# wangxiaohit/GNNPN-SC

Hardware: AMD Instinct MI355X
Metric: service-composition problems/sec (ML+2PN inference) (higher is better)
Workload: dtype f32-split3xf16 (f32 operands and results; recurrent W_hh.h products: fp32 operands split exactly into 3 x f16, six f16-matrix-core products per term, f32 accumulate; everything else f32 arithmetic)

## Files before the change

gnnpn-sc_amd/csrc/decode_lean.hip:

```cpp
#include "common.h"
#include "recurrent.h"
#include "decode_shared.h"
#include "coop_common.h"
#include "lstm_shared.h"

namespace {
constexpr int H = COOP_H;
constexpr int G = COOP_G;
constexpr int ROWS = COOP_ROWS;
constexpr int UNITS = H / G;
constexpr int KW = 16;
constexpr unsigned SPIN_LIMIT = 400000;
constexpr int XP_GRANULES = ROWS * KW * G;

typedef unsigned u32x2 __attribute__((ext_vector_type(2)));
constexpr int AUX_SC1 = 16;


__device__ __forceinline__ __amdgpu_buffer_rsrc_t make_rsrc(const void* p, unsigned bytes) {
    return __builtin_amdgcn_make_buffer_rsrc(const_cast<void*>(p), 0, (int)bytes, 0x00020000);
}
__device__ __forceinline__ void store_granule(__amdgpu_buffer_rsrc_t r, unsigned voff, unsigned soff, u64 g, bool same_xcd) {
    const u32x2 v = {(unsigned)g, (unsigned)(g >> 32)};
    if (same_xcd) __builtin_amdgcn_raw_buffer_store_b64(v, r, voff, soff, 0);
    else __builtin_amdgcn_raw_buffer_store_b64(v, r, voff, soff, AUX_SC1);
}
}

template <bool SPLIT, int OCC, int EVH, bool DIAG = false>
__global__ __launch_bounds__(256, OCC) void pointer_decode_lean_kernel(DecodeArgs a, u64* xh, u64* xp,
                                                                     u64* xl, unsigned* __restrict__ err,
                                                                     unsigned* __restrict__ sticky, int n_nets, int groups_per_net,
                                                                     int gpx, int flags, unsigned* __restrict__ seats,
                                                                     unsigned* __restrict__ diag) {
    __shared__ __attribute__((aligned(16))) float hs[SPLIT ? 3 * SPLIT_TILE / 2 : ROWS * LDT];
    __shared__ __attribute__((aligned(16))) unsigned wts[SPLIT ? SPLIT_WT_DWORDS : 4];
    __shared__ __attribute__((aligned(16))) float hsl[ROWS][UNITS + 4];
    __shared__ __attribute__((aligned(16))) float win[ROWS][KW][8];
    __shared__ int sel[ROWS];
    __shared__ int abort_flag;
    __shared__ int place[2];

    const int tid = threadIdx.x, lane = tid & 63, wave = __builtin_amdgcn_readfirstlane(tid >> 6);
    const int kq = lane >> 4, c = lane & 15;
    CoopSeat seat;
    if (!coop_enter<G>(err, sticky, seats, gpx, flags, n_nets, groups_per_net, place, &abort_flag, seat)) return;
    const int group = __builtin_amdgcn_readfirstlane(seat.group), member = __builtin_amdgcn_readfirstlane(seat.member);
    const int net_id = __builtin_amdgcn_readfirstlane(seat.net), gi = __builtin_amdgcn_readfirstlane(seat.index_in_net);
    const bool same_xcd = seat.same_xcd;
    const DecodeNet& net = a.net[net_id];

    const int B = a.B, T = a.T, K = a.K, L = T * K;
    const bool latent_in_launch = net.latent_from >= 0;
    const bool has_lat = latent_in_launch || net.latent_win;
    bool publishes_latent = false;
    for (int n = 0; n < n_nets; ++n) publishes_latent |= (a.net[n].latent_from == net_id);
    const bool first = member == 0;

    const int unit = member * UNITS + wave * 8 + (c & 7);
    const int wrow[2] = {(0 + (c >> 3)) * H + unit, (2 + (c >> 3)) * H + unit};
    float wBh[SPLIT ? 1 : 2][SPLIT ? 1 : 64];
    f16x8 wH16[SPLIT ? 2 : 1][8], wL16[SPLIT ? 2 : 1][8];
    float winv[2] = {1.0f, 1.0f};
    unsigned* wt_lane = wts + (SPLIT ? (wave * 8 * 64 + lane) * 4 : 0);
    float bh[2], bi[2], sg[2], wXf[2][2];
    const uint4* __restrict__ Wsplit = SPLIT ? static_cast<const uint4*>(net.whh_split) : nullptr;
    if constexpr (SPLIT) {
        if (Wsplit) load_split_weights(Wsplit + (size_t)member * SPLIT_PACK_U4_PER_MEMBER, tid, wH16, wL16, wt_lane, winv);
    }
#pragma unroll
    for (int tl = 0; tl < 2; ++tl) {
        const int gate = wrow[tl] / H, u = wrow[tl] % H;
        bh[tl] = net.bhh[wrow[tl]];
        if constexpr (SPLIT) {
            if (!Wsplit) winv[tl] = split_weights<H>(net.whh, gate, u, kq, wH16[tl], wL16[tl], wt_lane + 2 * tl);
        } else {
            load_whh_fragments<H>(net.whh, gate, u, kq, wBh[tl]);
        }
        load_folded_input(net.xw_fold, net.xb_fold, wrow[tl], kq, wXf[tl], bi[tl]);
        sg[tl] = net.start_fold[wrow[tl]];
    }

    const int own0 = kq * 4 + (c < 8 ? 0 : 2);
    const int vo_hpub = (int)(own0 * H + unit) * 8u;
    const int vo_sweep = 16 * lane;
    constexpr int VO_NONE = (int)0xFFFFFF00u;
    const int rq = kq, r = c;
    const bool live = r < K;
    const int vo_p = live ? 64 * lane : VO_NONE;
    const int vo_lat = live ? (int)(rq * K + r) * 8u : VO_NONE;
    const int vo_wl = (int)((wave * 4 + rq) * T * K + r) * 4u;
    const int vo_idx = (int)((wave * 4 + rq) * T) * 4u;
    const int vo_act = (int)(c * T * 8 + kq) * 4u;
    const int vo_q = (int)(own0 * T * H + unit) * 4u;
    constexpr int EVN = 8 / EVH;
    const int ppair = tid / EVH, phalf = tid - ppair * EVH;
    const int prow = ppair / K, pcand = ppair - prow * K;
    const bool pdot = ppair < ROWS * K;
    const int vo_ev = pdot ? (int)(((size_t)prow * L + pcand) * H + member * UNITS + phalf * (4 * EVN)) * 4u : VO_NONE;
    const int vo_ppub = (int)((prow * KW + pcand) * G + member) * 8u;
    const int wr_row = tid >> 4, wr_cand = tid & 15;
    const bool wr_live = wr_cand < K;
    const int vo_win = wr_live ? (int)(((size_t)wr_row * L + wr_cand) * 8) * 4u : VO_NONE;

    __amdgpu_buffer_rsrc_t r_h = make_rsrc(xh + (size_t)group * (2 * ROWS * H), 2 * ROWS * H * 8);
    __amdgpu_buffer_rsrc_t r_p = make_rsrc(xp + (size_t)group * (2 * XP_GRANULES), 2 * XP_GRANULES * 8);

    const int n_tiles = (B + ROWS - 1) / ROWS;
    unsigned step = 0;
    unsigned tiles_done = 0;
    for (int tile = gi; tile < n_tiles; tile += groups_per_net) {
        const int b0 = tile * ROWS;
        const int rows_here = min(ROWS, B - b0);
        __amdgpu_buffer_rsrc_t r_enc = make_rsrc(net.enc_out + (size_t)b0 * L * H, (unsigned)((size_t)rows_here * L * H * 4));
        __amdgpu_buffer_rsrc_t r_in = make_rsrc(a.inputs + (size_t)b0 * L * 8, (unsigned)((size_t)rows_here * L * 32));
        __amdgpu_buffer_rsrc_t r_lat = make_rsrc(xl + (size_t)tile * T * ROWS * K, (unsigned)((size_t)T * ROWS * K * 8));
        __amdgpu_buffer_rsrc_t r_wl = make_rsrc(net.win_logits + (size_t)b0 * T * K, (unsigned)((size_t)rows_here * T * K * 4));
        __amdgpu_buffer_rsrc_t r_idx = make_rsrc(net.idx + (size_t)b0 * T, (unsigned)((size_t)rows_here * T * 4));
        __amdgpu_buffer_rsrc_t r_act = make_rsrc(net.actions + (size_t)b0 * T * 8, (unsigned)((size_t)rows_here * T * 32));
        __amdgpu_buffer_rsrc_t r_lw = make_rsrc(net.latent_win ? net.latent_win + (size_t)b0 * T * K : nullptr,
                                                net.latent_win ? (unsigned)((size_t)rows_here * T * K * 4) : 0u);
        __amdgpu_buffer_rsrc_t r_q = make_rsrc(net.queries ? net.queries + (size_t)b0 * T * H : nullptr,
                                               net.queries ? (unsigned)((size_t)rows_here * T * H * 4) : 0u);
        f32x2 cst, hl = {0.f, 0.f};
        cst.x = b0 + own0 < B ? net.c0[(int64_t)(b0 + own0) * H + unit] : 0.0f;
        cst.y = b0 + own0 + 1 < B ? net.c0[(int64_t)(b0 + own0 + 1) * H + unit] : 0.0f;
        __syncthreads();
        for (int j = 0; j < ROWS; ++j) {
            const float h0v = (b0 + j < B) ? net.h0[(int64_t)(b0 + j) * H + tid] : 0.0f;
            if constexpr (SPLIT) split_store(reinterpret_cast<_Float16*>(hs) + j * LDH16 + tid, h0v);
            else hs[ht_index(j, tid)] = h0v;
        }
        __syncthreads();

        for (int k = 0; k <= T; ++k) {
            float axf0 = 0.0f, axf1 = 0.0f;
            u64 st[8] = {0, 0, 0, 0, 0, 0, 0, 0};
            if constexpr (DIAG) st[0] = st[1] = st[2] = st[3] = st[4] = st[5] = phase_stamp();
            const unsigned tag = step;
            const unsigned par = (step - 1) & 1;
            const unsigned so_k = (unsigned)k * (unsigned)K;
            u32x4 ev[EVN];
            u32x4 vp[4];
            u32x2 vl;
#pragma unroll
            for (int j = 0; j < EVN; ++j) asm volatile("" : "=v"(ev[j]));
#pragma unroll
            for (int j = 0; j < 4; ++j) asm volatile("" : "=v"(vp[j]));
            asm volatile("" : "=v"(vl));
            f32x4 ah[2] = {f32x4{0.f, 0.f, 0.f, 0.f}, f32x4{0.f, 0.f, 0.f, 0.f}};

            constexpr bool EV_EARLY = OCC == 1;
            auto request_ev = [&]() {
#pragma unroll
                for (int j = 0; j < EVN; ++j) ev[j] = __builtin_amdgcn_raw_buffer_load_b128(r_enc, vo_ev, so_k * (H * 4) + 16u * j, 0);
            };
            if (k < T) {
                if (k > 0) {
                    const unsigned so_h0 = par * (ROWS * H * 8) + wave * (4 * H * 8);
                    u32x4 vh[8];
                    bool ok = false;
                    unsigned h_miss = 0;
                    for (unsigned spins = 0; spins <= SPIN_LIMIT; ++spins) {
                        unsigned so_h = so_h0;
                        asm volatile("" : "+s"(so_h));
#pragma unroll
                        for (int j = 0; j < 8; ++j) vh[j] = __builtin_amdgcn_raw_buffer_load_b128(r_h, vo_sweep, so_h + 1024u * j, AUX_SC1);
                        bool good = true;
#pragma unroll
                        for (int j = 0; j < 8; ++j) {
                            if constexpr (SPLIT) good &= split_pair_tagged(vh[j], tag);
                            else good &= (vh[j].y == tag) & (vh[j].w == tag);
                        }
                        if (__all(good)) {
                            ok = true;
                            break;
                        }
                        __builtin_amdgcn_s_sleep(1);
                    }
                    if constexpr (DIAG) st[1] = phase_stamp();
                    if (!ok) {
                        abort_flag = 1;
#pragma unroll
                        for (int j = 0; j < 8; ++j) {
                            bool bad;
                            if constexpr (SPLIT) bad = !split_pair_tagged(vh[j], tag);
                            else bad = (vh[j].y != tag) | (vh[j].w != tag);
                            const unsigned long long bm = __ballot(bad);
                            for (int q = 0; q < 4; ++q)
                                if ((bm >> (16 * q)) & 0xffffull) h_miss |= 1u << (4 * (j & 1) + q);
                        }
                        if (lane == 0) coop_failure_record(diag, err, gpx, group, member, tile, k, wave, tag, h_miss, 0u, 0u);
                    }
#pragma unroll
                    for (int j = 0; j < 8; ++j) {
                        const int i = 2 * (j * 64 + lane);
                        if constexpr (SPLIT) {
                            split_pair_to_lds(reinterpret_cast<_Float16*>(hs) + (wave * 4 + (i >> 8)) * LDH16 + (i & 255), vh[j]);
                        } else {
                            float* d = &hs[ht_index(wave * 4 + (i >> 8), i & 255)];
                            d[0] = __uint_as_float(vh[j].x);
                            d[64] = __uint_as_float(vh[j].z);
                        }
                    }
                    if constexpr (EV_EARLY) request_ev();
                    __syncthreads();
                    if (abort_flag) break;
                } else if constexpr (EV_EARLY) {
                    request_ev();
                }
                if constexpr (DIAG) st[2] = phase_stamp();
                constexpr bool EARLY_P = OCC == 1 || !SPLIT;
                auto request_p = [&]() {
                    if (EARLY_P && k > 0) {
                        const unsigned so_p = par * (XP_GRANULES * 8) + wave * (4 * KW * G * 8);
#pragma unroll
                        for (int j = 0; j < 4; ++j) vp[j] = __builtin_amdgcn_raw_buffer_load_b128(r_p, vo_p, so_p + 16u * j, AUX_SC1);
                        if (latent_in_launch)
                            vl = __builtin_amdgcn_raw_buffer_load_b64(r_lat, vo_lat, (unsigned)(((k - 1) * ROWS + wave * 4) * K) * 8u, AUX_SC1);
                    }
                };
                if constexpr (SPLIT) split_chain(reinterpret_cast<const _Float16*>(hs) + c * LDH16 + 8 * kq, wH16, wL16, wt_lane, winv, ah, request_p);
                else mfma_chain_pair<LDT, OCC == 2 ? 8 : 16, true>(hs, c, kq, wBh[0], wBh[SPLIT ? 0 : 1], ah[0], ah[1], request_p);
                if constexpr (DIAG) {
                    asm volatile("" ::"v"(ah[0][0]), "v"(ah[1][0]));
                    st[3] = phase_stamp();
                }
            }

            if (k > 0) {
                const unsigned so_p0 = par * (XP_GRANULES * 8) + wave * (4 * KW * G * 8);
                const unsigned so_l0 = (unsigned)(((k - 1) * ROWS + wave * 4) * K) * 8u;
                bool ok = false;
                for (unsigned spins = 0; spins <= SPIN_LIMIT; ++spins) {
                    if (spins > 0 || k == T || (OCC != 1 && SPLIT)) {
                        unsigned so_p = so_p0, so_l = so_l0;
                        asm volatile("" : "+s"(so_p), "+s"(so_l));
#pragma unroll
                        for (int j = 0; j < 4; ++j) vp[j] = __builtin_amdgcn_raw_buffer_load_b128(r_p, vo_p, so_p + 16u * j, AUX_SC1);
                        if (latent_in_launch) vl = __builtin_amdgcn_raw_buffer_load_b64(r_lat, vo_lat, so_l, AUX_SC1);
                    }
                    bool good = true;
                    if (live) {
#pragma unroll
                        for (int j = 0; j < 4; ++j) good &= (vp[j].y == tag) & (vp[j].w == tag);
                        if (latent_in_launch) good &= vl.y == 1u;
                    }
                    if (__all(good)) {
                        ok = true;
                        break;
                    }
                    __builtin_amdgcn_s_sleep(1);
                }
                if constexpr (DIAG) st[4] = phase_stamp();
                if (!ok) {
                    abort_flag = 1;
                    unsigned p_miss = 0;
#pragma unroll
                    for (int j = 0; j < 4; ++j) {
                        if (__ballot(live && vp[j].y != tag)) p_miss |= 1u << (2 * j);
                        if (__ballot(live && vp[j].w != tag)) p_miss |= 1u << (2 * j + 1);
                    }
                    const unsigned l_miss = (unsigned)__popcll(__ballot(live && latent_in_launch && vl.y != 1u));
                    if (lane == 0) coop_failure_record(diag, err, gpx, group, member, tile, k, wave, tag, 0u, p_miss, l_miss);
                }

                {
                    const int row = wave * 4 + rq;
                    const unsigned so_t = (unsigned)(k - 1) * (unsigned)K * 4u;
                    float dot = 0.0f, lv = 0.0f;
                    if (live) {
                        dot = __fadd_rn(__fadd_rn(__fadd_rn(__uint_as_float(vp[0].x), __uint_as_float(vp[0].z)), __uint_as_float(vp[1].x)), __uint_as_float(vp[1].z));
                        dot = __fadd_rn(__fadd_rn(__fadd_rn(__fadd_rn(dot, __uint_as_float(vp[2].x)), __uint_as_float(vp[2].z)), __uint_as_float(vp[3].x)), __uint_as_float(vp[3].z));
                        if (latent_in_launch) lv = __uint_as_float(vl.x);
                        else if (net.latent_win) lv = __uint_as_float(__builtin_amdgcn_raw_buffer_load_b32(r_lw, vo_wl, so_t, 0));
                    }
                    float v = a.use_tanh ? __fmul_rn(a.tanh_c, tanhf(dot)) : dot;
                    if (live && first) {
                        __builtin_amdgcn_raw_buffer_store_b32(__float_as_uint(v), r_wl, vo_wl, so_t, 0);
                        if (publishes_latent)
                            __builtin_amdgcn_raw_buffer_store_b64(u32x2{__float_as_uint(v), 1u}, r_lat, vo_lat, so_l0, AUX_SC1);
                    }
                    v = (has_lat && live) ? __fadd_rn(v, lv) : v;
                    float m = live ? v : -INFINITY;
                    m = fmaxf(m, dpp_ror16(m, 8));
                    m = fmaxf(m, dpp_ror16(m, 4));
                    m = fmaxf(m, dpp_ror16(m, 2));
                    m = fmaxf(m, dpp_ror16(m, 1));
                    const unsigned hit = (unsigned)(__ballot(live && v == m) >> (16 * rq)) & 0xffffu;
                    const int pick_r = hit ? __ffs(hit) - 1 : 0;
                    if (r == 0) {
                        sel[row] = pick_r;
                        if (first) __builtin_amdgcn_raw_buffer_store_b32((unsigned)((k - 1) * K + pick_r), r_idx, vo_idx, (unsigned)(k - 1) * 4u, 0);
                    }
                }
                __syncthreads();
                if (abort_flag) break;
                axf0 = win[c][sel[c]][kq];
                axf1 = win[c][sel[c]][4 + kq];
                if (first && wave == 0) {
                    __builtin_amdgcn_raw_buffer_store_b32(__float_as_uint(axf0), r_act, vo_act, (unsigned)(k - 1) * 32u, 0);
                    __builtin_amdgcn_raw_buffer_store_b32(__float_as_uint(axf1), r_act, vo_act, (unsigned)(k - 1) * 32u + 16u, 0);
                }
                if (k == T) break;
                if constexpr (DIAG) st[5] = phase_stamp();
            }

            if constexpr (!EV_EARLY) request_ev();
            u32x4 wv0, wv1;
            wv0 = __builtin_amdgcn_raw_buffer_load_b128(r_in, vo_win, so_k * 32u, 0);
            wv1 = __builtin_amdgcn_raw_buffer_load_b128(r_in, vo_win, so_k * 32u + 16u, 0);
            float gx[2][4];
            if (k > 0) {
                f32x4 ax0 = {0.f, 0.f, 0.f, 0.f}, ax1 = ax0;
                ax0 = __builtin_amdgcn_mfma_f32_16x16x4f32(axf0, wXf[0][0], ax0, 0, 0, 0);
                ax1 = __builtin_amdgcn_mfma_f32_16x16x4f32(axf0, wXf[1][0], ax1, 0, 0, 0);
                ax0 = __builtin_amdgcn_mfma_f32_16x16x4f32(axf1, wXf[0][1], ax0, 0, 0, 0);
                ax1 = __builtin_amdgcn_mfma_f32_16x16x4f32(axf1, wXf[1][1], ax1, 0, 0, 0);
#pragma unroll
                for (int q = 0; q < 4; ++q) {
                    gx[0][q] = __fadd_rn(ax0[q], bi[0]);
                    gx[1][q] = __fadd_rn(ax1[q], bi[1]);
                }
            } else {
#pragma unroll
                for (int q = 0; q < 4; ++q) {
                    gx[0][q] = sg[0];
                    gx[1][q] = sg[1];
                }
            }
            {
                f32x2 g0[2], g1[2];
                gates_before_cell(ah[0], ah[1], bh, gx, g0, g1);
                cell_update_split(g0, g1, c < 8, cst, hl);
            }
            {
                const unsigned so_pub = (step & 1) * (ROWS * H * 8);
                if constexpr (SPLIT) {
                    store_granule(r_h, vo_hpub, so_pub, split_granule(step + 1, hl.x), same_xcd);
                    store_granule(r_h, vo_hpub, so_pub + H * 8, split_granule(step + 1, hl.y), same_xcd);
                } else {
                    store_granule(r_h, vo_hpub, so_pub, ((u64)(step + 1) << 32) | __float_as_uint(hl.x), same_xcd);
                    store_granule(r_h, vo_hpub, so_pub + H * 8, ((u64)(step + 1) << 32) | __float_as_uint(hl.y), same_xcd);
                }
                hsl[own0][wave * 8 + (c & 7)] = hl.x;
                hsl[own0 + 1][wave * 8 + (c & 7)] = hl.y;
                if (net.queries) {
                    __builtin_amdgcn_raw_buffer_store_b32(__float_as_uint(hl.x), r_q, vo_q, (unsigned)k * (H * 4), 0);
                    __builtin_amdgcn_raw_buffer_store_b32(__float_as_uint(hl.y), r_q, vo_q, (unsigned)(k + T) * (H * 4), 0);
                }
            }
            if constexpr (DIAG) {
                asm volatile("" ::"v"(hl.y));
                st[6] = phase_stamp();
            }
            __syncthreads();
            {
                float p = 0.0f;
                if (pdot) {
#pragma unroll
                    for (int j = 0; j < EVN; ++j) {
                        const float4 hv = *reinterpret_cast<const float4*>(&hsl[prow][phalf * (4 * EVN) + 4 * j]);
                        p = fmaf(__uint_as_float(ev[j].x), hv.x, p);
                        p = fmaf(__uint_as_float(ev[j].y), hv.y, p);
                        p = fmaf(__uint_as_float(ev[j].z), hv.z, p);
                        p = fmaf(__uint_as_float(ev[j].w), hv.w, p);
                    }
                }
                if constexpr (EVH == 2)
                    p = __fadd_rn(p, __int_as_float(__builtin_amdgcn_update_dpp(0, __float_as_int(p), 0xB1 , 0xF, 0xF, false)));
                if (pdot && phalf == 0)
                    store_granule(r_p, vo_ppub, (step & 1) * (XP_GRANULES * 8), ((u64)(step + 1) << 32) | __float_as_uint(p), same_xcd);
            }
            if (wr_live) {
                *reinterpret_cast<u32x4*>(&win[wr_row][wr_cand][0]) = wv0;
                *reinterpret_cast<u32x4*>(&win[wr_row][wr_cand][4]) = wv1;
            }
            if constexpr (DIAG) {
                st[7] = phase_stamp();
                if (blockIdx.x == 0 && tid == 0 && k > 0) {
                    u64* prof = reinterpret_cast<u64*>(err) + 4;
                    prof[0] += st[1] - st[0];
                    prof[1] += st[2] - st[1];
                    prof[2] += st[3] - st[2];
                    prof[3] += st[4] - st[3];
                    prof[4] += st[5] - st[4];
                    prof[5] += st[6] - st[5];
                    prof[6] += st[7] - st[6];
                    prof[7] += 1;
                }
            }
            ++step;
        }
        if (abort_flag) break;
        ++tiles_done;
    }
    coop_leave(err, sticky, seats, abort_flag, 2u, GNNPN_STATUS_DEC_FINISHED, tiles_done);
}

struct PickProbArgs {
    const float* win[2];
    const float* lat[2];
    const int32_t* idx[2];
    float* out[2];
};
__global__ __launch_bounds__(256) void pick_prob_kernel(PickProbArgs a, int64_t rows, int T, int K) {
    const int net = blockIdx.y;
    const float* __restrict__ win = a.win[net];
    const float* __restrict__ lat = a.lat[net];
    const int32_t* __restrict__ idx = a.idx[net];
    float* __restrict__ out = a.out[net];
    const int64_t row = blockIdx.x * 256ll + threadIdx.x;
    if (row >= rows) return;
    const unsigned t_base = (unsigned)__builtin_amdgcn_readfirstlane((int)((blockIdx.x * 256ll) % T));
    const int t = (int)((t_base + threadIdx.x) % (unsigned)T);
    float v[16];
#pragma unroll
    for (int j = 0; j < 16; ++j) {
        v[j] = 0.0f;
        if (j < K) {
            v[j] = win[row * K + j];
            if (lat) v[j] = __fadd_rn(v[j], lat[row * K + j]);
        }
    }
    const int pick_r = min(max(idx[row] - t * K, 0), 15);
    float best = v[0];
#pragma unroll
    for (int j = 1; j < 16; ++j) best = j == pick_r ? v[j] : best;
#pragma unroll
    for (int j = 0; j < 16; ++j) v[j] = j < K ? expf(__fsub_rn(v[j], best)) : 0.0f;
#pragma unroll
    for (int n = 8; n >= 1; n >>= 1)
#pragma unroll
        for (int j = 0; j < n; ++j) v[j] = __fadd_rn(v[j], v[j + n]);
    out[row] = 1.0f / v[0];
}

static DecodeWorkspace lean_workspace(int64_t groups, int64_t rows, int32_t T, int32_t K) {
    return decode_workspace(groups, rows, T, K, XP_GRANULES);
}

int64_t gnnpn_decode_lean_workspace_bytes(int32_t B, int32_t T, int32_t n_per) { return lean_workspace(64, B, T, n_per).total(); }

int gnnpn_launch_decode_lean(const DecodeArgs& args, int n_nets, int precision, bool shared_cu, const CoopOpts& opts,
                             void* workspace, int64_t workspace_bytes, hipStream_t s) {
    if (args.K > KW) GNNPN_FAIL(GNNPN_E_UNSUP, "pointer_decode: the cooperative form is built for n_per <= %d", KW);
    if ((int64_t)ROWS * args.T * args.K * H * 4 >= (1ll << 32) || (int64_t)args.T * ROWS * args.K * 8 >= (1ll << 32))
        GNNPN_FAIL(GNNPN_E_UNSUP, "pointer_decode: a tile of 16 problems must stay below 4 GB of encoder output");
    const bool split = precision == GNNPN_PREC_SPLIT;
    const bool wide = args.K > 8;
    const bool stamps = (gnnpn_option_lstm_ablate() & GNNPN_ABLATE_DEC_STAMPS) != 0;
    if (stamps && wide) GNNPN_FAIL(GNNPN_E_UNSUP, "pointer_decode: the stamped build exists for n_per <= 8");
    CoopLaunch c;
    const auto need = [&](int groups) { return lean_workspace(groups, args.B, args.T, args.K).total(); };
    if (const int rc = coop_begin("pointer_decode", n_nets, args.B, need, GNNPN_STATUS_DEC_EXPECTED, opts, workspace, workspace_bytes, s, c))
        return rc;
    const DecodeWorkspace w = lean_workspace(c.groups, args.B, args.T, args.K);
#define GNNPN_LEAN(SPLIT_, OCC_, EVH_, ...)                                                                                           \
    hipLaunchKernelGGL((pointer_decode_lean_kernel<SPLIT_, OCC_, EVH_, ##__VA_ARGS__>), dim3(COOP_OVERSUB * c.groups * G), dim3(256),       \
                       gnnpn_lds_padding((const void*)pointer_decode_lean_kernel<SPLIT_, OCC_, EVH_, ##__VA_ARGS__>, opts.lds_kb), s, args, \
                       w.h(c.buffers), w.p(c.buffers), w.l(c.buffers), c.status, opts.sticky, n_nets, c.groups_per_net, c.gpx, coop_flags(opts), c.seats, c.diag)
    if (stamps) {
        if (split) GNNPN_LEAN(true, 1, 2, true);
        else GNNPN_LEAN(false, 1, 2, true);
    } else if (split && shared_cu && wide) GNNPN_LEAN(true, 2, 1);
    else if (split && shared_cu) GNNPN_LEAN(true, 2, 2);
    else if (split && wide) GNNPN_LEAN(true, 1, 1);
    else if (split) GNNPN_LEAN(true, 1, 2);
    else if (shared_cu && wide) GNNPN_LEAN(false, 2, 1);
    else if (shared_cu) GNNPN_LEAN(false, 2, 2);
    else if (wide) GNNPN_LEAN(false, 1, 1);
    else GNNPN_LEAN(false, 1, 2);
#undef GNNPN_LEAN
    if (hipGetLastError() != hipSuccess) GNNPN_FAIL(GNNPN_E_LAUNCH, "pointer_decode: launch of the cooperative kernel failed");
    const int64_t rows = (int64_t)args.B * args.T;
    for (int n0 = 0; n0 < n_nets; n0 += 2) {
        PickProbArgs pa = {};
        const int cnt = n_nets - n0 < 2 ? n_nets - n0 : 2;
        for (int n = 0; n < cnt; ++n) {
            const DecodeNet& d = args.net[n0 + n];
            pa.win[n] = d.win_logits;
            pa.lat[n] = d.latent_from >= 0 ? args.net[d.latent_from].win_logits : d.latent_win;
            pa.idx[n] = d.idx;
            pa.out[n] = d.pick_prob;
        }
        hipLaunchKernelGGL(pick_prob_kernel, dim3((unsigned)((rows + 255) / 256), (unsigned)cnt), dim3(256), 0, s, pa, rows, args.T, args.K);
    }
    return GNNPN_OK;
}
```

Before: 488,900.

## Specialize lean decode kernel per member role and step kind at compile time

Moves the per-tile decode loop into a device function templated on latent mode, publisher, first-member and queries flags, dispatched once per block by a switch on the runtime role. The first, middle and last decode steps become separate compile-time variants, so per-step branches on k and on net flags disappear, and unused buffer descriptors are not built. The h and p exchange buffers are merged into one buffer resource addressed by a scalar offset, saving scalar registers. The cost is many more kernel instantiations, longer compile time and larger code, which may pressure the instruction cache.

```diff
diff --git a/gnnpn-sc_amd/csrc/decode_lean.hip b/gnnpn-sc_amd/csrc/decode_lean.hip
--- a/gnnpn-sc_amd/csrc/decode_lean.hip
+++ b/gnnpn-sc_amd/csrc/decode_lean.hip
@@ -20,66 +20,55 @@
 __device__ __forceinline__ __amdgpu_buffer_rsrc_t make_rsrc(const void* p, unsigned bytes) {
     return __builtin_amdgcn_make_buffer_rsrc(const_cast<void*>(p), 0, (int)bytes, 0x00020000);
 }
-__device__ __forceinline__ void store_granule(__amdgpu_buffer_rsrc_t r, unsigned voff, unsigned soff, u64 g, bool same_xcd) {
+__device__ __forceinline__ void store_granule(__amdgpu_buffer_rsrc_t r, unsigned voff, unsigned soff, u64 g, int same_xcd) {
     const u32x2 v = {(unsigned)g, (unsigned)(g >> 32)};
+    asm volatile("" : "+s"(same_xcd));
     if (same_xcd) __builtin_amdgcn_raw_buffer_store_b64(v, r, voff, soff, 0);
     else __builtin_amdgcn_raw_buffer_store_b64(v, r, voff, soff, AUX_SC1);
 }
-}
-
-template <bool SPLIT, int OCC, int EVH, bool DIAG = false>
-__global__ __launch_bounds__(256, OCC) void pointer_decode_lean_kernel(DecodeArgs a, u64* xh, u64* xp,
-                                                                     u64* xl, unsigned* __restrict__ err,
-                                                                     unsigned* __restrict__ sticky, int n_nets, int groups_per_net,
-                                                                     int gpx, int flags, unsigned* __restrict__ seats,
-                                                                     unsigned* __restrict__ diag) {
-    __shared__ __attribute__((aligned(16))) float hs[SPLIT ? 3 * SPLIT_TILE / 2 : ROWS * LDT];
-    __shared__ __attribute__((aligned(16))) unsigned wts[SPLIT ? SPLIT_WT_DWORDS : 4];
-    __shared__ __attribute__((aligned(16))) float hsl[ROWS][UNITS + 4];
-    __shared__ __attribute__((aligned(16))) float win[ROWS][KW][8];
-    __shared__ int sel[ROWS];
-    __shared__ int abort_flag;
-    __shared__ int place[2];
-
-    const int tid = threadIdx.x, lane = tid & 63, wave = __builtin_amdgcn_readfirstlane(tid >> 6);
-    const int kq = lane >> 4, c = lane & 15;
-    CoopSeat seat;
-    if (!coop_enter<G>(err, sticky, seats, gpx, flags, n_nets, groups_per_net, place, &abort_flag, seat)) return;
-    const int group = __builtin_amdgcn_readfirstlane(seat.group), member = __builtin_amdgcn_readfirstlane(seat.member);
-    const int net_id = __builtin_amdgcn_readfirstlane(seat.net), gi = __builtin_amdgcn_readfirstlane(seat.index_in_net);
-    const bool same_xcd = seat.same_xcd;
-    const DecodeNet& net = a.net[net_id];
-
-    const int B = a.B, T = a.T, K = a.K, L = T * K;
-    const bool latent_in_launch = net.latent_from >= 0;
-    const bool has_lat = latent_in_launch || net.latent_win;
-    bool publishes_latent = false;
-    for (int n = 0; n < n_nets; ++n) publishes_latent |= (a.net[n].latent_from == net_id);
-    const bool first = member == 0;
-
-    const int unit = member * UNITS + wave * 8 + (c & 7);
-    const int wrow[2] = {(0 + (c >> 3)) * H + unit, (2 + (c >> 3)) * H + unit};
+
+enum : int { LAT_NONE = 0, LAT_LAUNCH = 1, LAT_STORED = 2 };
+enum : int { STEP_FIRST = 0, STEP_MID = 1, STEP_LAST = 2 };
+template <int V>
+struct StepKind {
+    static constexpr int value = V;
+};
+
+template <bool SPLIT>
+struct LeanWeights {
     float wBh[SPLIT ? 1 : 2][SPLIT ? 1 : 64];
     f16x8 wH16[SPLIT ? 2 : 1][8], wL16[SPLIT ? 2 : 1][8];
-    float winv[2] = {1.0f, 1.0f};
-    unsigned* wt_lane = wts + (SPLIT ? (wave * 8 * 64 + lane) * 4 : 0);
+    float winv[2];
+    unsigned* wt_lane;
     float bh[2], bi[2], sg[2], wXf[2][2];
-    const uint4* __restrict__ Wsplit = SPLIT ? static_cast<const uint4*>(net.whh_split) : nullptr;
-    if constexpr (SPLIT) {
-        if (Wsplit) load_split_weights(Wsplit + (size_t)member * SPLIT_PACK_U4_PER_MEMBER, tid, wH16, wL16, wt_lane, winv);
-    }
-#pragma unroll
-    for (int tl = 0; tl < 2; ++tl) {
-        const int gate = wrow[tl] / H, u = wrow[tl] % H;
-        bh[tl] = net.bhh[wrow[tl]];
-        if constexpr (SPLIT) {
-            if (!Wsplit) winv[tl] = split_weights<H>(net.whh, gate, u, kq, wH16[tl], wL16[tl], wt_lane + 2 * tl);
-        } else {
-            load_whh_fragments<H>(net.whh, gate, u, kq, wBh[tl]);
-        }
-        load_folded_input(net.xw_fold, net.xb_fold, wrow[tl], kq, wXf[tl], bi[tl]);
-        sg[tl] = net.start_fold[wrow[tl]];
-    }
+};
+struct LeanLds {
+    float* hs;
+    float (*hsl)[UNITS + 4];
+    float (*win)[KW][8];
+    int* sel;
+    int* abort_flag;
+};
+struct LeanSeat {
+    int group, member, gi, wave;
+    int same_xcd;
+};
+
+template <bool SPLIT, int OCC, int EVH, bool DIAG, int LAT, bool PUB, bool FIRST, bool QUERIES>
+__device__ __forceinline__ unsigned lean_member_tiles(const DecodeArgs& a, const DecodeNet& net, u64* xh, u64* xp, u64* xl,
+                                                      unsigned* __restrict__ err, unsigned* __restrict__ diag, int gpx,
+                                                      int groups_per_net, const LeanSeat seat, const LeanWeights<SPLIT>& w,
+                                                      const LeanLds lds, const int unit) {
+    static_assert(!PUB || FIRST, "only member 0 publishes the window logits");
+    static_assert(!(PUB && LAT == LAT_LAUNCH), "a net that reads another net's logits is the last of the launch");
+    const int tid = threadIdx.x, lane = tid & 63, wave = seat.wave;
+    const int kq = lane >> 4, c = lane & 15;
+    const int group = seat.group, member = seat.member;
+    const int same_xcd = seat.same_xcd;
+    float* const hs = lds.hs;
+    const int B = a.B, T = a.T, K = a.K, L = T * K;
+    constexpr bool HAS_LAT = LAT != LAT_NONE;
+    constexpr bool USES_XL = LAT == LAT_LAUNCH || PUB;
 
     const int own0 = kq * 4 + (c < 8 ? 0 : 2);
     const int vo_hpub = (int)(own0 * H + unit) * 8u;
@@ -100,28 +89,32 @@
     const int vo_ev = pdot ? (int)(((size_t)prow * L + pcand) * H + member * UNITS + phalf * (4 * EVN)) * 4u : VO_NONE;
     const int vo_ppub = (int)((prow * KW + pcand) * G + member) * 8u;
     const int wr_row = tid >> 4, wr_cand = tid & 15;
-    const bool wr_live = wr_cand < K;
+    const bool wr_live = live;
     const int vo_win = wr_live ? (int)(((size_t)wr_row * L + wr_cand) * 8) * 4u : VO_NONE;
 
-    __amdgpu_buffer_rsrc_t r_h = make_rsrc(xh + (size_t)group * (2 * ROWS * H), 2 * ROWS * H * 8);
-    __amdgpu_buffer_rsrc_t r_p = make_rsrc(xp + (size_t)group * (2 * XP_GRANULES), 2 * XP_GRANULES * 8);
+    const char* const xh_group = reinterpret_cast<const char*>(xh + (size_t)group * (2 * ROWS * H));
+    const unsigned so_xp = (unsigned)(reinterpret_cast<const char*>(xp + (size_t)group * (2 * XP_GRANULES)) - xh_group);
+    __amdgpu_buffer_rsrc_t r_x = make_rsrc(xh_group, so_xp + 2 * XP_GRANULES * 8);
 
     const int n_tiles = (B + ROWS - 1) / ROWS;
     unsigned step = 0;
     unsigned tiles_done = 0;
-    for (int tile = gi; tile < n_tiles; tile += groups_per_net) {
+    for (int tile = seat.gi; tile < n_tiles; tile += groups_per_net) {
         const int b0 = tile * ROWS;
         const int rows_here = min(ROWS, B - b0);
+        const __amdgpu_buffer_rsrc_t r_null = make_rsrc(nullptr, 0u);
         __amdgpu_buffer_rsrc_t r_enc = make_rsrc(net.enc_out + (size_t)b0 * L * H, (unsigned)((size_t)rows_here * L * H * 4));
         __amdgpu_buffer_rsrc_t r_in = make_rsrc(a.inputs + (size_t)b0 * L * 8, (unsigned)((size_t)rows_here * L * 32));
-        __amdgpu_buffer_rsrc_t r_lat = make_rsrc(xl + (size_t)tile * T * ROWS * K, (unsigned)((size_t)T * ROWS * K * 8));
-        __amdgpu_buffer_rsrc_t r_wl = make_rsrc(net.win_logits + (size_t)b0 * T * K, (unsigned)((size_t)rows_here * T * K * 4));
-        __amdgpu_buffer_rsrc_t r_idx = make_rsrc(net.idx + (size_t)b0 * T, (unsigned)((size_t)rows_here * T * 4));
-        __amdgpu_buffer_rsrc_t r_act = make_rsrc(net.actions + (size_t)b0 * T * 8, (unsigned)((size_t)rows_here * T * 32));
-        __amdgpu_buffer_rsrc_t r_lw = make_rsrc(net.latent_win ? net.latent_win + (size_t)b0 * T * K : nullptr,
-                                                net.latent_win ? (unsigned)((size_t)rows_here * T * K * 4) : 0u);
-        __amdgpu_buffer_rsrc_t r_q = make_rsrc(net.queries ? net.queries + (size_t)b0 * T * H : nullptr,
-                                               net.queries ? (unsigned)((size_t)rows_here * T * H * 4) : 0u);
+        __amdgpu_buffer_rsrc_t r_lat = r_null;
+        if constexpr (USES_XL) r_lat = make_rsrc(xl + (size_t)tile * T * ROWS * K, (unsigned)((size_t)T * ROWS * K * 8));
+        __amdgpu_buffer_rsrc_t r_wl = r_null, r_idx = r_null, r_act = r_null, r_lw = r_null, r_q = r_null;
+        if constexpr (FIRST) {
+            r_wl = make_rsrc(net.win_logits + (size_t)b0 * T * K, (unsigned)((size_t)rows_here * T * K * 4));
+            r_idx = make_rsrc(net.idx + (size_t)b0 * T, (unsigned)((size_t)rows_here * T * 4));
+            r_act = make_rsrc(net.actions + (size_t)b0 * T * 8, (unsigned)((size_t)rows_here * T * 32));
+        }
+        if constexpr (LAT == LAT_STORED) r_lw = make_rsrc(net.latent_win + (size_t)b0 * T * K, (unsigned)((size_t)rows_here * T * K * 4));
+        if constexpr (QUERIES) r_q = make_rsrc(net.queries + (size_t)b0 * T * H, (unsigned)((size_t)rows_here * T * H * 4));
         f32x2 cst, hl = {0.f, 0.f};
         cst.x = b0 + own0 < B ? net.c0[(int64_t)(b0 + own0) * H + unit] : 0.0f;
         cst.y = b0 + own0 + 1 < B ? net.c0[(int64_t)(b0 + own0 + 1) * H + unit] : 0.0f;
@@ -133,21 +126,29 @@
         }
         __syncthreads();
 
-        for (int k = 0; k <= T; ++k) {
+        auto decode_step = [&](auto kind, const int k) __attribute__((always_inline)) -> bool {
+            constexpr int KIND = decltype(kind)::value;
+            constexpr bool SWEEPS = KIND != STEP_FIRST;
+            constexpr bool ADVANCES = KIND != STEP_LAST;
+            constexpr bool STAMPS = DIAG && KIND == STEP_MID;
             float axf0 = 0.0f, axf1 = 0.0f;
             u64 st[8] = {0, 0, 0, 0, 0, 0, 0, 0};
-            if constexpr (DIAG) st[0] = st[1] = st[2] = st[3] = st[4] = st[5] = phase_stamp();
+            if constexpr (STAMPS) st[0] = st[1] = st[2] = st[3] = st[4] = st[5] = phase_stamp();
             const unsigned tag = step;
             const unsigned par = (step - 1) & 1;
             const unsigned so_k = (unsigned)k * (unsigned)K;
             u32x4 ev[EVN];
             u32x4 vp[4];
             u32x2 vl;
-#pragma unroll
-            for (int j = 0; j < EVN; ++j) asm volatile("" : "=v"(ev[j]));
-#pragma unroll
-            for (int j = 0; j < 4; ++j) asm volatile("" : "=v"(vp[j]));
-            asm volatile("" : "=v"(vl));
+            if constexpr (ADVANCES) {
+#pragma unroll
+                for (int j = 0; j < EVN; ++j) asm volatile("" : "=v"(ev[j]));
+            }
+            if constexpr (SWEEPS) {
+#pragma unroll
+                for (int j = 0; j < 4; ++j) asm volatile("" : "=v"(vp[j]));
+                if constexpr (LAT == LAT_LAUNCH) asm volatile("" : "=v"(vl));
+            }
             f32x4 ah[2] = {f32x4{0.f, 0.f, 0.f, 0.f}, f32x4{0.f, 0.f, 0.f, 0.f}};
 
             constexpr bool EV_EARLY = OCC == 1;
@@ -155,8 +156,8 @@
 #pragma unroll
                 for (int j = 0; j < EVN; ++j) ev[j] = __builtin_amdgcn_raw_buffer_load_b128(r_enc, vo_ev, so_k * (H * 4) + 16u * j, 0);
             };
-            if (k < T) {
-                if (k > 0) {
+            if constexpr (ADVANCES) {
+                if constexpr (SWEEPS) {
                     const unsigned so_h0 = par * (ROWS * H * 8) + wave * (4 * H * 8);
                     u32x4 vh[8];
                     bool ok = false;
@@ -165,7 +166,7 @@
                         unsigned so_h = so_h0;
                         asm volatile("" : "+s"(so_h));
 #pragma unroll
-                        for (int j = 0; j < 8; ++j) vh[j] = __builtin_amdgcn_raw_buffer_load_b128(r_h, vo_sweep, so_h + 1024u * j, AUX_SC1);
+                        for (int j = 0; j < 8; ++j) vh[j] = __builtin_amdgcn_raw_buffer_load_b128(r_x, vo_sweep, so_h + 1024u * j, AUX_SC1);
                         bool good = true;
 #pragma unroll
                         for (int j = 0; j < 8; ++j) {
@@ -178,9 +179,9 @@
                         }
                         __builtin_amdgcn_s_sleep(1);
                     }
-                    if constexpr (DIAG) st[1] = phase_stamp();
+                    if constexpr (STAMPS) st[1] = phase_stamp();
                     if (!ok) {
-                        abort_flag = 1;
+                        *lds.abort_flag = 1;
 #pragma unroll
                         for (int j = 0; j < 8; ++j) {
                             bool bad;
@@ -205,46 +206,47 @@
                     }
                     if constexpr (EV_EARLY) request_ev();
                     __syncthreads();
-                    if (abort_flag) break;
+                    if (__builtin_amdgcn_readfirstlane(*lds.abort_flag)) return false;
                 } else if constexpr (EV_EARLY) {
                     request_ev();
                 }
-                if constexpr (DIAG) st[2] = phase_stamp();
+                if constexpr (STAMPS) st[2] = phase_stamp();
                 constexpr bool EARLY_P = OCC == 1 || !SPLIT;
                 auto request_p = [&]() {
-                    if (EARLY_P && k > 0) {
-                        const unsigned so_p = par * (XP_GRANULES * 8) + wave * (4 * KW * G * 8);
-#pragma unroll
-                        for (int j = 0; j < 4; ++j) vp[j] = __builtin_amdgcn_raw_buffer_load_b128(r_p, vo_p, so_p + 16u * j, AUX_SC1);
-                        if (latent_in_launch)
+                    if constexpr (EARLY_P && SWEEPS) {
+                        const unsigned so_p = so_xp + par * (XP_GRANULES * 8) + wave * (4 * KW * G * 8);
+#pragma unroll
+                        for (int j = 0; j < 4; ++j) vp[j] = __builtin_amdgcn_raw_buffer_load_b128(r_x, vo_p, so_p + 16u * j, AUX_SC1);
+                        if constexpr (LAT == LAT_LAUNCH)
                             vl = __builtin_amdgcn_raw_buffer_load_b64(r_lat, vo_lat, (unsigned)(((k - 1) * ROWS + wave * 4) * K) * 8u, AUX_SC1);
                     }
                 };
-                if constexpr (SPLIT) split_chain(reinterpret_cast<const _Float16*>(hs) + c * LDH16 + 8 * kq, wH16, wL16, wt_lane, winv, ah, request_p);
-                else mfma_chain_pair<LDT, OCC == 2 ? 8 : 16, true>(hs, c, kq, wBh[0], wBh[SPLIT ? 0 : 1], ah[0], ah[1], request_p);
-                if constexpr (DIAG) {
+                if constexpr (SPLIT) split_chain(reinterpret_cast<const _Float16*>(hs) + c * LDH16 + 8 * kq, w.wH16, w.wL16, w.wt_lane, w.winv, ah, request_p);
+                else mfma_chain_pair<LDT, OCC == 2 ? 8 : 16, true>(hs, c, kq, w.wBh[0], w.wBh[SPLIT ? 0 : 1], ah[0], ah[1], request_p);
+                if constexpr (STAMPS) {
                     asm volatile("" ::"v"(ah[0][0]), "v"(ah[1][0]));
                     st[3] = phase_stamp();
                 }
             }
 
-            if (k > 0) {
-                const unsigned so_p0 = par * (XP_GRANULES * 8) + wave * (4 * KW * G * 8);
+            if constexpr (SWEEPS) {
+                constexpr bool EARLY_P = ADVANCES && (OCC == 1 || !SPLIT);
+                const unsigned so_p0 = so_xp + par * (XP_GRANULES * 8) + wave * (4 * KW * G * 8);
                 const unsigned so_l0 = (unsigned)(((k - 1) * ROWS + wave * 4) * K) * 8u;
                 bool ok = false;
                 for (unsigned spins = 0; spins <= SPIN_LIMIT; ++spins) {
-                    if (spins > 0 || k == T || (OCC != 1 && SPLIT)) {
+                    if (spins > 0 || !EARLY_P) {
                         unsigned so_p = so_p0, so_l = so_l0;
                         asm volatile("" : "+s"(so_p), "+s"(so_l));
 #pragma unroll
-                        for (int j = 0; j < 4; ++j) vp[j] = __builtin_amdgcn_raw_buffer_load_b128(r_p, vo_p, so_p + 16u * j, AUX_SC1);
-                        if (latent_in_launch) vl = __builtin_amdgcn_raw_buffer_load_b64(r_lat, vo_lat, so_l, AUX_SC1);
+                        for (int j = 0; j < 4; ++j) vp[j] = __builtin_amdgcn_raw_buffer_load_b128(r_x, vo_p, so_p + 16u * j, AUX_SC1);
+                        if constexpr (LAT == LAT_LAUNCH) vl = __builtin_amdgcn_raw_buffer_load_b64(r_lat, vo_lat, so_l, AUX_SC1);
                     }
                     bool good = true;
                     if (live) {
 #pragma unroll
                         for (int j = 0; j < 4; ++j) good &= (vp[j].y == tag) & (vp[j].w == tag);
-                        if (latent_in_launch) good &= vl.y == 1u;
+                        if constexpr (LAT == LAT_LAUNCH) good &= vl.y == 1u;
                     }
                     if (__all(good)) {
                         ok = true;
@@ -252,16 +254,17 @@
                     }
                     __builtin_amdgcn_s_sleep(1);
                 }
-                if constexpr (DIAG) st[4] = phase_stamp();
+                if constexpr (STAMPS) st[4] = phase_stamp();
                 if (!ok) {
-                    abort_flag = 1;
+                    *lds.abort_flag = 1;
                     unsigned p_miss = 0;
 #pragma unroll
                     for (int j = 0; j < 4; ++j) {
                         if (__ballot(live && vp[j].y != tag)) p_miss |= 1u << (2 * j);
                         if (__ballot(live && vp[j].w != tag)) p_miss |= 1u << (2 * j + 1);
                     }
-                    const unsigned l_miss = (unsigned)__popcll(__ballot(live && latent_in_launch && vl.y != 1u));
+                    unsigned l_miss = 0u;
+                    if constexpr (LAT == LAT_LAUNCH) l_miss = (unsigned)__popcll(__ballot(live && vl.y != 1u));
                     if (lane == 0) coop_failure_record(diag, err, gpx, group, member, tile, k, wave, tag, 0u, p_miss, l_miss);
                 }
 
@@ -272,16 +275,18 @@
                     if (live) {
                         dot = __fadd_rn(__fadd_rn(__fadd_rn(__uint_as_float(vp[0].x), __uint_as_float(vp[0].z)), __uint_as_float(vp[1].x)), __uint_as_float(vp[1].z));
                         dot = __fadd_rn(__fadd_rn(__fadd_rn(__fadd_rn(dot, __uint_as_float(vp[2].x)), __uint_as_float(vp[2].z)), __uint_as_float(vp[3].x)), __uint_as_float(vp[3].z));
-                        if (latent_in_launch) lv = __uint_as_float(vl.x);
-                        else if (net.latent_win) lv = __uint_as_float(__builtin_amdgcn_raw_buffer_load_b32(r_lw, vo_wl, so_t, 0));
+                        if constexpr (LAT == LAT_LAUNCH) lv = __uint_as_float(vl.x);
+                        else if constexpr (LAT == LAT_STORED) lv = __uint_as_float(__builtin_amdgcn_raw_buffer_load_b32(r_lw, vo_wl, so_t, 0));
                     }
                     float v = a.use_tanh ? __fmul_rn(a.tanh_c, tanhf(dot)) : dot;
-                    if (live && first) {
-                        __builtin_amdgcn_raw_buffer_store_b32(__float_as_uint(v), r_wl, vo_wl, so_t, 0);
-                        if (publishes_latent)
-                            __builtin_amdgcn_raw_buffer_store_b64(u32x2{__float_as_uint(v), 1u}, r_lat, vo_lat, so_l0, AUX_SC1);
-                    }
-                    v = (has_lat && live) ? __fadd_rn(v, lv) : v;
+                    if constexpr (FIRST) {
+                        if (live) {
+                            __builtin_amdgcn_raw_buffer_store_b32(__float_as_uint(v), r_wl, vo_wl, so_t, 0);
+                            if constexpr (PUB)
+                                __builtin_amdgcn_raw_buffer_store_b64(u32x2{__float_as_uint(v), 1u}, r_lat, vo_lat, so_l0, AUX_SC1);
+                        }
+                    }
+                    if constexpr (HAS_LAT) v = live ? __fadd_rn(v, lv) : v;
                     float m = live ? v : -INFINITY;
                     m = fmaxf(m, dpp_ror16(m, 8));
                     m = fmaxf(m, dpp_ror16(m, 4));
@@ -290,111 +295,201 @@
                     const unsigned hit = (unsigned)(__ballot(live && v == m) >> (16 * rq)) & 0xffffu;
                     const int pick_r = hit ? __ffs(hit) - 1 : 0;
                     if (r == 0) {
-                        sel[row] = pick_r;
-                        if (first) __builtin_amdgcn_raw_buffer_store_b32((unsigned)((k - 1) * K + pick_r), r_idx, vo_idx, (unsigned)(k - 1) * 4u, 0);
+                        lds.sel[row] = pick_r;
+                        if constexpr (FIRST) __builtin_amdgcn_raw_buffer_store_b32((unsigned)((k - 1) * K + pick_r), r_idx, vo_idx, (unsigned)(k - 1) * 4u, 0);
                     }
                 }
                 __syncthreads();
-                if (abort_flag) break;
-                axf0 = win[c][sel[c]][kq];
-                axf1 = win[c][sel[c]][4 + kq];
-                if (first && wave == 0) {
-                    __builtin_amdgcn_raw_buffer_store_b32(__float_as_uint(axf0), r_act, vo_act, (unsigned)(k - 1) * 32u, 0);
-                    __builtin_amdgcn_raw_buffer_store_b32(__float_as_uint(axf1), r_act, vo_act, (unsigned)(k - 1) * 32u + 16u, 0);
-                }
-                if (k == T) break;
-                if constexpr (DIAG) st[5] = phase_stamp();
+                if (__builtin_amdgcn_readfirstlane(*lds.abort_flag)) return false;
+                axf0 = lds.win[c][lds.sel[c]][kq];
+                axf1 = lds.win[c][lds.sel[c]][4 + kq];
+                if constexpr (FIRST) {
+                    if (wave == 0) {
+                        __builtin_amdgcn_raw_buffer_store_b32(__float_as_uint(axf0), r_act, vo_act, (unsigned)(k - 1) * 32u, 0);
+                        __builtin_amdgcn_raw_buffer_store_b32(__float_as_uint(axf1), r_act, vo_act, (unsigned)(k - 1) * 32u + 16u, 0);
+                    }
+                }
+                if constexpr (STAMPS) st[5] = phase_stamp();
             }
 
-            if constexpr (!EV_EARLY) request_ev();
-            u32x4 wv0, wv1;
-            wv0 = __builtin_amdgcn_raw_buffer_load_b128(r_in, vo_win, so_k * 32u, 0);
-            wv1 = __builtin_amdgcn_raw_buffer_load_b128(r_in, vo_win, so_k * 32u + 16u, 0);
-            float gx[2][4];
-            if (k > 0) {
-                f32x4 ax0 = {0.f, 0.f, 0.f, 0.f}, ax1 = ax0;
-                ax0 = __builtin_amdgcn_mfma_f32_16x16x4f32(axf0, wXf[0][0], ax0, 0, 0, 0);
-                ax1 = __builtin_amdgcn_mfma_f32_16x16x4f32(axf0, wXf[1][0], ax1, 0, 0, 0);
-                ax0 = __builtin_amdgcn_mfma_f32_16x16x4f32(axf1, wXf[0][1], ax0, 0, 0, 0);
-                ax1 = __builtin_amdgcn_mfma_f32_16x16x4f32(axf1, wXf[1][1], ax1, 0, 0, 0);
-#pragma unroll
-                for (int q = 0; q < 4; ++q) {
-                    gx[0][q] = __fadd_rn(ax0[q], bi[0]);
-                    gx[1][q] = __fadd_rn(ax1[q], bi[1]);
-                }
-            } else {
-#pragma unroll
-                for (int q = 0; q < 4; ++q) {
-                    gx[0][q] = sg[0];
-                    gx[1][q] = sg[1];
-                }
+            if constexpr (ADVANCES) {
+                if constexpr (!EV_EARLY) request_ev();
+                u32x4 wv0, wv1;
+                wv0 = __builtin_amdgcn_raw_buffer_load_b128(r_in, vo_win, so_k * 32u, 0);
+                wv1 = __builtin_amdgcn_raw_buffer_load_b128(r_in, vo_win, so_k * 32u + 16u, 0);
+                float gx[2][4];
+                if constexpr (SWEEPS) {
+                    f32x4 ax0 = {0.f, 0.f, 0.f, 0.f}, ax1 = ax0;
+                    ax0 = __builtin_amdgcn_mfma_f32_16x16x4f32(axf0, w.wXf[0][0], ax0, 0, 0, 0);
+                    ax1 = __builtin_amdgcn_mfma_f32_16x16x4f32(axf0, w.wXf[1][0], ax1, 0, 0, 0);
+                    ax0 = __builtin_amdgcn_mfma_f32_16x16x4f32(axf1, w.wXf[0][1], ax0, 0, 0, 0);
+                    ax1 = __builtin_amdgcn_mfma_f32_16x16x4f32(axf1, w.wXf[1][1], ax1, 0, 0, 0);
+#pragma unroll
+                    for (int q = 0; q < 4; ++q) {
+                        gx[0][q] = __fadd_rn(ax0[q], w.bi[0]);
+                        gx[1][q] = __fadd_rn(ax1[q], w.bi[1]);
+                    }
+                } else {
+#pragma unroll
+                    for (int q = 0; q < 4; ++q) {
+                        gx[0][q] = w.sg[0];
+                        gx[1][q] = w.sg[1];
+                    }
+                }
+                {
+                    f32x2 g0[2], g1[2];
+                    gates_before_cell(ah[0], ah[1], w.bh, gx, g0, g1);
+                    cell_update_split(g0, g1, c < 8, cst, hl);
+                }
+                {
+                    const unsigned so_pub = (step & 1) * (ROWS * H * 8);
+                    if constexpr (SPLIT) {
+                        store_granule(r_x, vo_hpub, so_pub, split_granule(step + 1, hl.x), same_xcd);
+                        store_granule(r_x, vo_hpub, so_pub + H * 8, split_granule(step + 1, hl.y), same_xcd);
+                    } else {
+                        store_granule(r_x, vo_hpub, so_pub, ((u64)(step + 1) << 32) | __float_as_uint(hl.x), same_xcd);
+                        store_granule(r_x, vo_hpub, so_pub + H * 8, ((u64)(step + 1) << 32) | __float_as_uint(hl.y), same_xcd);
+                    }
+                    lds.hsl[own0][wave * 8 + (c & 7)] = hl.x;
+                    lds.hsl[own0 + 1][wave * 8 + (c & 7)] = hl.y;
+                    if constexpr (QUERIES) {
+                        __builtin_amdgcn_raw_buffer_store_b32(__float_as_uint(hl.x), r_q, vo_q, (unsigned)k * (H * 4), 0);
+                        __builtin_amdgcn_raw_buffer_store_b32(__float_as_uint(hl.y), r_q, vo_q, (unsigned)(k + T) * (H * 4), 0);
+                    }
+                }
+                if constexpr (STAMPS) {
+                    asm volatile("" ::"v"(hl.y));
+                    st[6] = phase_stamp();
+                }
+                __syncthreads();
+                {
+                    float p = 0.0f;
+                    if (pdot) {
+#pragma unroll
+                        for (int j = 0; j < EVN; ++j) {
+                            const float4 hv = *reinterpret_cast<const float4*>(&lds.hsl[prow][phalf * (4 * EVN) + 4 * j]);
+                            p = fmaf(__uint_as_float(ev[j].x), hv.x, p);
+                            p = fmaf(__uint_as_float(ev[j].y), hv.y, p);
+                            p = fmaf(__uint_as_float(ev[j].z), hv.z, p);
+                            p = fmaf(__uint_as_float(ev[j].w), hv.w, p);
+                        }
+                    }
+                    if constexpr (EVH == 2)
+                        p = __fadd_rn(p, __int_as_float(__builtin_amdgcn_update_dpp(0, __float_as_int(p), 0xB1 , 0xF, 0xF, false)));
+                    if (pdot && phalf == 0)
+                        store_granule(r_x, vo_ppub, so_xp + (step & 1) * (XP_GRANULES * 8), ((u64)(step + 1) << 32) | __float_as_uint(p), same_xcd);
+                }
+                if (wr_live) {
+                    *reinterpret_cast<u32x4*>(&lds.win[wr_row][wr_cand][0]) = wv0;
+                    *reinterpret_cast<u32x4*>(&lds.win[wr_row][wr_cand][4]) = wv1;
+                }
+                if constexpr (STAMPS) {
+                    st[7] = phase_stamp();
+                    if (blockIdx.x == 0 && tid == 0) {
+                        u64* prof = reinterpret_cast<u64*>(err) + 4;
+                        prof[0] += st[1] - st[0];
+                        prof[1] += st[2] - st[1];
+                        prof[2] += st[3] - st[2];
+                        prof[3] += st[4] - st[3];
+                        prof[4] += st[5] - st[4];
+                        prof[5] += st[6] - st[5];
+                        prof[6] += st[7] - st[6];
+                        prof[7] += 1;
+                    }
+                }
+                ++step;
             }
-            {
-                f32x2 g0[2], g1[2];
-                gates_before_cell(ah[0], ah[1], bh, gx, g0, g1);
-                cell_update_split(g0, g1, c < 8, cst, hl);
-            }
-            {
-                const unsigned so_pub = (step & 1) * (ROWS * H * 8);
-                if constexpr (SPLIT) {
-                    store_granule(r_h, vo_hpub, so_pub, split_granule(step + 1, hl.x), same_xcd);
-                    store_granule(r_h, vo_hpub, so_pub + H * 8, split_granule(step + 1, hl.y), same_xcd);
-                } else {
-                    store_granule(r_h, vo_hpub, so_pub, ((u64)(step + 1) << 32) | __float_as_uint(hl.x), same_xcd);
-                    store_granule(r_h, vo_hpub, so_pub + H * 8, ((u64)(step + 1) << 32) | __float_as_uint(hl.y), same_xcd);
-                }
-                hsl[own0][wave * 8 + (c & 7)] = hl.x;
-                hsl[own0 + 1][wave * 8 + (c & 7)] = hl.y;
-                if (net.queries) {
-                    __builtin_amdgcn_raw_buffer_store_b32(__float_as_uint(hl.x), r_q, vo_q, (unsigned)k * (H * 4), 0);
-                    __builtin_amdgcn_raw_buffer_store_b32(__float_as_uint(hl.y), r_q, vo_q, (unsigned)(k + T) * (H * 4), 0);
-                }
-            }
-            if constexpr (DIAG) {
-                asm volatile("" ::"v"(hl.y));
-                st[6] = phase_stamp();
-            }
-            __syncthreads();
-            {
-                float p = 0.0f;
-                if (pdot) {
-#pragma unroll
-                    for (int j = 0; j < EVN; ++j) {
-                        const float4 hv = *reinterpret_cast<const float4*>(&hsl[prow][phalf * (4 * EVN) + 4 * j]);
-                        p = fmaf(__uint_as_float(ev[j].x), hv.x, p);
-                        p = fmaf(__uint_as_float(ev[j].y), hv.y, p);
-                        p = fmaf(__uint_as_float(ev[j].z), hv.z, p);
-                        p = fmaf(__uint_as_float(ev[j].w), hv.w, p);
-                    }
-                }
-                if constexpr (EVH == 2)
-                    p = __fadd_rn(p, __int_as_float(__builtin_amdgcn_update_dpp(0, __float_as_int(p), 0xB1 , 0xF, 0xF, false)));
-                if (pdot && phalf == 0)
-                    store_granule(r_p, vo_ppub, (step & 1) * (XP_GRANULES * 8), ((u64)(step + 1) << 32) | __float_as_uint(p), same_xcd);
-            }
-            if (wr_live) {
-                *reinterpret_cast<u32x4*>(&win[wr_row][wr_cand][0]) = wv0;
-                *reinterpret_cast<u32x4*>(&win[wr_row][wr_cand][4]) = wv1;
-            }
-            if constexpr (DIAG) {
-                st[7] = phase_stamp();
-                if (blockIdx.x == 0 && tid == 0 && k > 0) {
-                    u64* prof = reinterpret_cast<u64*>(err) + 4;
-                    prof[0] += st[1] - st[0];
-                    prof[1] += st[2] - st[1];
-                    prof[2] += st[3] - st[2];
-                    prof[3] += st[4] - st[3];
-                    prof[4] += st[5] - st[4];
-                    prof[5] += st[6] - st[5];
-                    prof[6] += st[7] - st[6];
-                    prof[7] += 1;
-                }
-            }
-            ++step;
-        }
-        if (abort_flag) break;
+            return true;
+        };
+
+        bool alive = decode_step(StepKind<STEP_FIRST>{}, 0);
+        for (int k = 1; alive && k < T; ++k) alive = decode_step(StepKind<STEP_MID>{}, k);
+        if (alive) alive = decode_step(StepKind<STEP_LAST>{}, T);
+        if (!alive) break;
         ++tiles_done;
     }
+    return tiles_done;
+}
+}
+
+template <bool SPLIT, int OCC, int EVH, bool DIAG = false>
+__global__ __launch_bounds__(256, OCC) void pointer_decode_lean_kernel(DecodeArgs a, u64* xh, u64* xp,
+                                                                     u64* xl, unsigned* __restrict__ err,
+                                                                     unsigned* __restrict__ sticky, int n_nets, int groups_per_net,
+                                                                     int gpx, int flags, unsigned* __restrict__ seats,
+                                                                     unsigned* __restrict__ diag) {
+    __shared__ __attribute__((aligned(16))) float hs[SPLIT ? 3 * SPLIT_TILE / 2 : ROWS * LDT];
+    __shared__ __attribute__((aligned(16))) unsigned wts[SPLIT ? SPLIT_WT_DWORDS : 4];
+    __shared__ __attribute__((aligned(16))) float hsl[ROWS][UNITS + 4];
+    __shared__ __attribute__((aligned(16))) float win[ROWS][KW][8];
+    __shared__ int sel[ROWS];
+    __shared__ int abort_flag;
+    __shared__ int place[2];
+
+    const int tid = threadIdx.x, lane = tid & 63, wave = __builtin_amdgcn_readfirstlane(tid >> 6);
+    const int kq = lane >> 4, c = lane & 15;
+    CoopSeat seat;
+    if (!coop_enter<G>(err, sticky, seats, gpx, flags, n_nets, groups_per_net, place, &abort_flag, seat)) return;
+    const int group = __builtin_amdgcn_readfirstlane(seat.group), member = __builtin_amdgcn_readfirstlane(seat.member);
+    const int net_id = __builtin_amdgcn_readfirstlane(seat.net), gi = __builtin_amdgcn_readfirstlane(seat.index_in_net);
+    const DecodeNet& net = a.net[net_id];
+
+    const int unit = member * UNITS + wave * 8 + (c & 7);
+    const int wrow[2] = {(0 + (c >> 3)) * H + unit, (2 + (c >> 3)) * H + unit};
+    LeanWeights<SPLIT> w;
+    w.winv[0] = w.winv[1] = 1.0f;
+    w.wt_lane = wts + (SPLIT ? (wave * 8 * 64 + lane) * 4 : 0);
+    const uint4* __restrict__ Wsplit = SPLIT ? static_cast<const uint4*>(net.whh_split) : nullptr;
+    if constexpr (SPLIT) {
+        if (Wsplit) load_split_weights(Wsplit + (size_t)member * SPLIT_PACK_U4_PER_MEMBER, tid, w.wH16, w.wL16, w.wt_lane, w.winv);
+    }
+#pragma unroll
+    for (int tl = 0; tl < 2; ++tl) {
+        const int gate = wrow[tl] / H, u = wrow[tl] % H;
+        w.bh[tl] = net.bhh[wrow[tl]];
+        if constexpr (SPLIT) {
+            if (!Wsplit) w.winv[tl] = split_weights<H>(net.whh, gate, u, kq, w.wH16[tl], w.wL16[tl], w.wt_lane + 2 * tl);
+        } else {
+            load_whh_fragments<H>(net.whh, gate, u, kq, w.wBh[tl]);
+        }
+        load_folded_input(net.xw_fold, net.xb_fold, wrow[tl], kq, w.wXf[tl], w.bi[tl]);
+        w.sg[tl] = net.start_fold[wrow[tl]];
+    }
+
+    bool publishes_latent = false;
+    for (int n = 0; n < n_nets; ++n) publishes_latent |= (a.net[n].latent_from == net_id);
+    const int lat = net.latent_from >= 0 ? LAT_LAUNCH : net.latent_win ? LAT_STORED : LAT_NONE;
+    const bool first = member == 0;
+    const int role = lat | (first ? 4 : 0) | (first && publishes_latent ? 8 : 0) | (net.queries ? 16 : 0);
+    const LeanSeat ls = {group, member, gi, wave, seat.same_xcd ? 1 : 0};
+    const LeanLds lds = {hs, hsl, win, sel, &abort_flag};
+    unsigned tiles_done = 0;
+#define GNNPN_ROLE(LAT_, PUB_, FIRST_, Q_)                                                                                       \
+    case (LAT_) | ((FIRST_) ? 4 : 0) | ((PUB_) ? 8 : 0) | ((Q_) ? 16 : 0):                                                         \
+        tiles_done = lean_member_tiles<SPLIT, OCC, EVH, DIAG, LAT_, PUB_, FIRST_, Q_>(a, net, xh, xp, xl, err, diag, gpx, groups_per_net, \
+                                                                                      ls, w, lds, unit);                          \
+        break;
+    switch (role) {
+        GNNPN_ROLE(LAT_NONE, false, false, false)
+        GNNPN_ROLE(LAT_LAUNCH, false, false, false)
+        GNNPN_ROLE(LAT_STORED, false, false, false)
+        GNNPN_ROLE(LAT_NONE, false, false, true)
+        GNNPN_ROLE(LAT_LAUNCH, false, false, true)
+        GNNPN_ROLE(LAT_STORED, false, false, true)
+        GNNPN_ROLE(LAT_NONE, false, true, false)
+        GNNPN_ROLE(LAT_LAUNCH, false, true, false)
+        GNNPN_ROLE(LAT_STORED, false, true, false)
+        GNNPN_ROLE(LAT_NONE, true, true, false)
+        GNNPN_ROLE(LAT_STORED, true, true, false)
+        GNNPN_ROLE(LAT_NONE, false, true, true)
+        GNNPN_ROLE(LAT_LAUNCH, false, true, true)
+        GNNPN_ROLE(LAT_STORED, false, true, true)
+        GNNPN_ROLE(LAT_NONE, true, true, true)
+        GNNPN_ROLE(LAT_STORED, true, true, true)
+    default:
+        break;
+    }
+#undef GNNPN_ROLE
     coop_leave(err, sticky, seats, abort_flag, 2u, GNNPN_STATUS_DEC_FINISHED, tiles_done);
 }
 
@@ -456,6 +551,7 @@
     if (const int rc = coop_begin("pointer_decode", n_nets, args.B, need, GNNPN_STATUS_DEC_EXPECTED, opts, workspace, workspace_bytes, s, c))
         return rc;
     const DecodeWorkspace w = lean_workspace(c.groups, args.B, args.T, args.K);
+    static_assert(64ll * 2 * (ROWS * H + XP_GRANULES) * 8 < (1ll << 31), "h and p granules of a launch within one buffer resource");
 #define GNNPN_LEAN(SPLIT_, OCC_, EVH_, ...)                                                                                           \
     hipLaunchKernelGGL((pointer_decode_lean_kernel<SPLIT_, OCC_, EVH_, ##__VA_ARGS__>), dim3(COOP_OVERSUB * c.groups * G), dim3(256),       \
                        gnnpn_lds_padding((const void*)pointer_decode_lean_kernel<SPLIT_, OCC_, EVH_, ##__VA_ARGS__>, opts.lds_kb), s, args, \
```

New measurement: 493,000 (median of 6 runs). Within noise of the previous version (+0.9%).
